# cheneeheng/2s-AGCN

Hardware: AMD Instinct MI355X
Metric: skeleton-clips/sec fwd+bwd, NTU (N,3,300,25,2) (higher is better)
Workload: dtype f32; 1 GPU; AGCN joint-stream NTU-xview shape, full training step (fwd, CE, bwd, grad all-reduce, clip 1.0, SGD nesterov); per_gpu_batch=64, global_batch=64, input=(N,3,300,25,2), parallelism=dp1, bn=per-replica

## Files before the change

### 2s-agcn_amd/csrc/gcn_chain.hip

```cpp
#include "agcn_common.h"
#include "split_f16.h"

namespace {

typedef __bf16 bf16x8 __attribute__((ext_vector_type(8)));
typedef __bf16 bf16x2 __attribute__((ext_vector_type(2)));
typedef float f32x2 __attribute__((ext_vector_type(2)));
typedef unsigned u32x4 __attribute__((ext_vector_type(4)));
typedef f32x4 f32x4_u __attribute__((aligned(4)));

constexpr int CB = 32;

struct ChainArgs {
  const float* in;
  const unsigned short* wp;
  const float* bias;
  float* out;
  const float* adj;
  float* stats;
  const float* add1;
  const float* mask1;
  const float* add2;
  const float* mask2;
  int N, M, K, T, V;
// ... 805 lines not shown
#pragma unroll
        for (int pl = 0; pl < 2; ++pl) af[pl] = *reinterpret_cast<const bf16x8*>(ab + ((pl * 2 + hf) * TM + tm) * 1024);
        acc[tm] = mfma3(af, gb[hf], acc[tm]);
      }
  };

  f32x4 xr[4];
  float dvb[16];
  const int t_first = f0 + wave;
  if (t_first < f1) load_x(t_first, 0, xr);
  __syncthreads();
  const unsigned long long tk_pro = (a.dbg & 8) ? wall_clock64() : 0;
  const unsigned long long ck_pro = (a.dbg & 8) ? clock64() : 0;

  long long ck_st = 0, ck_c = 0, ck_o = 0, ck_e = 0, ck0 = 0;
  int prev_t0 = -1;
  for (int t0 = f0; t0 < f1; t0 += WS_NW) {
    const int t = t0 + wave;
    const bool fvalid = t < f1 && !(a.dbg & 1);
    const bool nvalid_next = (t + WS_NW) < f1 && !(a.dbg & 2);
    f32x16 acc[TM];
#pragma unroll
    for (int tm = 0; tm < TM; ++tm)
#pragma unroll
      for (int j = 0; j < 16; ++j) acc[tm][j] = 0.f;
    if (a.dbg & 8) ck0 = clock64();
    if (fvalid) {
      if (NCB2 > 0) load_p(0, t, dvb);
      bf16x8 xq[2][2];
      u32x4 gw[2][2][2];
      bf16x8 bq[2][2];
      auto load_adj = [&](int i) __attribute__((always_inline)) {
        const unsigned char* aq = adjq + i * 2 * 2048 + (h * 32 + lr) * 16;
#pragma unroll
        for (int ks = 0; ks < 2; ++ks)
#pragma unroll
          for (int pl = 0; pl < 2; ++pl) bq[ks][pl] = *reinterpret_cast<const bf16x8*>(aq + pl * 2048 + ks * 1024);
      };
      auto agg = [&]() __attribute__((always_inline)) {
        f32x16 d;
#pragma unroll
        for (int j = 0; j < 16; ++j) d[j] = 0.f;
#pragma unroll
        for (int ks = 0; ks < 2; ++ks) d = mfma3(xq[ks], bq[ks], d);
        return d;
      };
      auto split_pairs = [&](const float (&dv)[16], int p0, int np, u32x4 (&gwn)[2][2], float sc) __attribute__((always_inline)) {
#pragma unroll
        for (int p = p0; p < p0 + np; ++p) {
          unsigned w0, w1;
          split_pair_f16_mix(dv[2 * p] * sc, dv[2 * p + 1] * sc, w0, w1);
          gwn[p >> 2][0][p & 3] = w0;
          gwn[p >> 2][1][p & 3] = w1;
        }
      };
      auto load_w = [&](int stage, int st, bf16x8 (&af)[2]) __attribute__((always_inline)) {
        const int hf = st / TM, tm = st - hf * TM;
        const unsigned char* ab = wimg + stage * A_IMG + lane * 16;
#pragma unroll
        for (int pl = 0; pl < 2; ++pl) af[pl] = *reinterpret_cast<const bf16x8*>(ab + ((pl * 2 + hf) * TM + tm) * 1024);
      };
      constexpr int NST = 2 * TM;
      constexpr int PP0[4] = {0, 0, 3, 6}, PPN[4] = {0, 3, 3, 2};
      constexpr int QP0[2] = {0, 0}, QPN[2] = {0, 8};
      splitx(xr, xq);
      if (KCB > 1) load_x(t, 1, xr);
      else if (nvalid_next) load_x(t + WS_NW, 0, xr);
      load_adj(0);
      {
        const f32x16 d = agg();
        load_adj(S1 > 1 ? 1 : 0);
        float dv[16];
#pragma unroll
        for (int j = 0; j < 16; ++j) dv[j] = d[j];
        split_pairs(dv, 0, 8, gw[0], 1.f);
      }
      bf16x8 afc[2], afn[2];
      load_w(0, 0, afc);
      __builtin_amdgcn_sched_barrier(0);
#pragma unroll
      for (int s = 0; s < S; ++s) {
        const int sn = s + 1;
        float dv[16];
        if (sn < S1) {
          if (sn % 3 == 0) {
            splitx(xr, xq);
            if (sn / 3 + 1 < KCB) load_x(t, sn / 3 + 1, xr);
            else if (nvalid_next) load_x(t + WS_NW, 0, xr);
          }
          const f32x16 dn = agg();
#pragma unroll
          for (int j = 0; j < 16; ++j) dv[j] = dn[j];
        } else if (sn < S) {
#pragma unroll
          for (int j = 0; j < 16; ++j) dv[j] = dvb[j];
        }
        __builtin_amdgcn_sched_barrier(0);
#pragma unroll
        for (int st = 0; st < NST; ++st) {
          if (!(a.dbg & 32)) {
            if (st + 1 < NST) load_w(s, st + 1, afn);
            else if (sn < S) load_w(sn, 0, afn);
          }
          if (st == NST - 2 && sn + 1 < S1 && !(a.dbg & 64)) load_adj((sn + 1) % 3);
          __builtin_amdgcn_sched_barrier(0);
          {
            const int hf = st / TM, tm = st - hf * TM;
            bf16x8 gbv[2] = {__builtin_bit_cast(bf16x8, gw[s & 1][hf][0]), __builtin_bit_cast(bf16x8, gw[s & 1][hf][1])};
            acc[tm] = mfma3(afc, gbv, acc[tm]);
          }
          if (sn < S && !(a.dbg & 16)) split_pairs(dv, NST == 4 ? PP0[st] : QP0[st], NST == 4 ? PPN[st] : QPN[st], gw[sn & 1], sn < S1 ? 1.f : rs_s);
          afc[0] = afn[0]; afc[1] = afn[1];
          __builtin_amdgcn_sched_barrier(0);
        }
        if (sn >= S1 && sn + 1 < S) load_p(sn + 1 - S1, t, dvb);
        if constexpr (!ROLES) {
          if (prev_t0 >= 0 && s * RB < RPW) {
            if (al16) store_rows_fast(O0, s * RB, prev_t0, WS_NW * V); else store_rows_slow(O0, s * RB, prev_t0, WS_NW * V);
          }
          __builtin_amdgcn_sched_barrier(0);
        }
      }
    }
    if constexpr (!ROLES) {
      if (prev_t0 >= 0 && !fvalid) store_tile(O0, prev_t0, WS_NW * V);
      prev_t0 = t0;
    }
    if (a.dbg & 8) { const long long c = clock64(); ck_st += c - ck0; ck0 = c; }
    if (o_stride == 0) asm volatile("s_waitcnt lgkmcnt(0)\n\ts_barrier" ::: "memory");
    if (a.dbg & 8) { const long long c = clock64(); ck_c += c - ck0; ck0 = c; }
    if (fvalid && lr < V) {
      float* O = O0 + (((t0 - f0) / WS_NW) & 1) * o_stride;
#pragma unroll
      for (int tm = 0; tm < TM; ++tm)
#pragma unroll
        for (int j = 0; j < 16; ++j) O[(tm * 32 + mfma_row(j, h)) * OPf + wave * V + lr] = acc[tm][j];
    }
    if (a.dbg & 8) { asm volatile("s_waitcnt lgkmcnt(0)" ::: "memory"); const long long c = clock64(); ck_o += c - ck0; ck0 = c; }
    asm volatile("s_waitcnt lgkmcnt(0)\n\ts_barrier" ::: "memory");
    if (a.dbg & 8) { const long long c = clock64(); ck_e += c - ck0; ck0 = c; }
  }
  const unsigned long long tk_loop = (a.dbg & 8) ? wall_clock64() : 0;
  if ((a.dbg & 8) && tid == 0) {
    float* o = a.out + blk0 + (long)f0 * V;
    o[0] = (float)(tk_pro - tk_entry); o[1] = (float)(tk_loop - tk_pro); o[2] = (float)(clock64() - ck_pro); o[3] = -12345.f;
    o[4] = (float)ck_st; o[5] = (float)ck_c; o[6] = (float)ck_o; o[7] = (float)ck_e;
  }
  if constexpr (!ROLES) {
    store_tile(O0, prev_t0, min(WS_NW, f1 - prev_t0) * V);
    store_stats();
  }
}

struct ChainGeom {
  int ntiles, ncb, nmb, XP, off_bias;
  size_t smem_bytes, pack_bytes;
};

template <int TM, int NW>
ChainGeom chain_geometry(int V, int T, int M, int K, bool bch = false, int planes = 3) {
  constexpr int BM = TM * 32, FT = NW;
  ChainGeom g;
  g.ntiles = (T + FT - 1) / FT;
  g.ncb = (K + CB - 1) / CB;
  g.nmb = (M + BM - 1) / BM;
  g.XP = (FT * V) | 1;
  const size_t a_img = (size_t)planes * 2 * TM * 1024;
  const size_t xb_bytes = ((size_t)CB * g.XP * 4 + (bch ? 128 : 0) + 15) & ~(size_t)15;
  g.smem_bytes = (bch ? (size_t)3 * planes * 2 * 2 * 32 * 16 : (size_t)3 * 32 * 32 * 4) + xb_bytes + 2 * a_img;
  const size_t epi_bytes = (size_t)BM * ((FT * V) | 1) * 4 + (size_t)NW * 64 * 2 * 4;
  if (epi_bytes > g.smem_bytes) g.smem_bytes = epi_bytes;
  g.smem_bytes = (g.smem_bytes + 15) & ~(size_t)15;
  g.off_bias = (int)g.smem_bytes;
  g.smem_bytes += (size_t)BM * 4;
  g.pack_bytes = (size_t)g.nmb * g.ncb * 3 * a_img;
  return g;
}

struct ChainW2 {
  const float* w;
  long sa_m, sa_c;
};

template <int TM, int VS, int NW, bool F16 = false>
int chain_launch(ChainArgs a, const float* w, long sa_m, long sa_i, long sa_c, const ChainW2& g_w2, void* ws,
                 size_t ws_bytes, hipStream_t stream) {
  constexpr int PL = F16 ? 2 : 3;
  const ChainGeom g = chain_geometry<TM, NW>(a.V, a.T, a.M, a.K, VS == 0, PL);
  if (g.smem_bytes > 160 * 1024) return AGCN_ERR_UNSUPPORTED;
  a.ncb2 = a.in2 ? (a.K2 + CB - 1) / CB : 0;
  const int s_total = 3 * g.ncb + a.ncb2;
  const size_t a_img = (size_t)PL * 2 * TM * 1024;
  const size_t img_bytes = (size_t)g.nmb * s_total * a_img;
  if (img_bytes + (F16 ? 16 : 0) > ws_bytes) return AGCN_ERR_WORKSPACE;
  if constexpr (F16) {
    unsigned* amax = reinterpret_cast<unsigned*>(static_cast<char*>(ws) + img_bytes);
    if (!a.in_absmax) {
      if (int rc = agcn_launch_absmax(a.in, (long)a.N * a.K * a.T * a.V, amax, stream)) return rc;
      a.in_absmax = reinterpret_cast<const float*>(amax);
    }
    if (a.in2 && !a.in2_absmax) {
      if (int rc = agcn_launch_absmax(a.in2, (long)a.N * a.K2 * a.T * a.V, amax + 1, stream)) return rc;
      a.in2_absmax = reinterpret_cast<const float*>(amax + 1);
    }
    if (!a.in2) a.in2_absmax = nullptr;
  }
  a.ntiles = g.ntiles; a.ncb = g.ncb; a.nmb = g.nmb; a.XP = g.XP; a.off_bias = g.off_bias;
  a.wp = (const unsigned short*)ws;
  ChainPackArgs pk;
  pk.w = w; pk.wp = (unsigned short*)ws; pk.M = a.M; pk.K = a.K; pk.ncb = g.ncb;
  pk.sa_m = sa_m; pk.sa_i = sa_i; pk.sa_c = sa_c;
  pk.nsub = 3; pk.s_total = s_total; pk.s_off = 0;
  hipLaunchKernelGGL((chain_pack_kernel<TM, F16>), dim3(g.nmb * g.ncb * 3), dim3(256), 0, stream, pk);
  int rc = agcn_check_launch();
  if (rc) return rc;
  if (a.ncb2 > 0) {
    ChainPackArgs p2;
    p2.w = g_w2.w; p2.wp = (unsigned short*)ws; p2.M = a.M; p2.K = a.K2; p2.ncb = a.ncb2;
    p2.sa_m = g_w2.sa_m; p2.sa_i = 0; p2.sa_c = g_w2.sa_c;
    p2.nsub = 1; p2.s_total = s_total; p2.s_off = 3 * g.ncb;
    hipLaunchKernelGGL((chain_pack_kernel<TM, F16>), dim3(g.nmb * a.ncb2), dim3(256), 0, stream, p2);
    rc = agcn_check_launch();
    if (rc) return rc;
  }
  auto kern = gcn_chain_kernel<TM, VS, NW, F16>;
  static unsigned char lds_ok[AGCN_MAX_DEVICES] = {};
  if (int e = agcn_allow_big_lds_rt(reinterpret_cast<const void*>(kern), lds_ok)) return e;
  hipLaunchKernelGGL(kern, dim3((unsigned)(a.N * g.ntiles * g.nmb)), dim3(NW * 64), g.smem_bytes, stream, a);
  AGCN_NOTE_KERNEL("gcn_chain_kernel<%d, %d, %d, %s>", TM, VS, NW, F16 ? "true" : "false");
  return agcn_check_launch();
}


static inline bool ws_enabled() {
  static const int on = getenv("AGCN_CHAIN_WS") ? atoi(getenv("AGCN_CHAIN_WS")) : 1;
  return on != 0;
}
static inline bool ws_shape_ok(int M, int K, int K2, int V) {
  if (!(agcn_chain_f16x3() && ws_enabled() && V <= 32 && M >= 1 && K > 32)) return false;
  static const int k128 = getenv("AGCN_WS_K128") ? atoi(getenv("AGCN_WS_K128")) : 1;
  return (K <= 64 && K2 >= 0 && K2 <= 96) || (k128 && K <= 128 && K2 == 0 && M > 32);
}

template <int TM, int NCB2, int KCB = 2>
int ws_launch(ChainArgs a, const float* w, long sa_m, long sa_i, long sa_c, const ChainW2& g_w2, void* ws, size_t ws_bytes,
              hipStream_t stream) {
  const WsGeom g = ws_geometry<TM>(a.N, a.M, a.K, a.K2, a.T, a.V);
  if (g.smem_bytes > 160 * 1024) return AGCN_ERR_UNSUPPORTED;
  if (NCB2 > 0 && a.stats) return AGCN_ERR_UNSUPPORTED;
  const size_t img_total = (size_t)g.nmb * g.img_bytes;
  if (img_total + 16 > ws_bytes) return AGCN_ERR_WORKSPACE;
  unsigned* amax = reinterpret_cast<unsigned*>(static_cast<char*>(ws) + img_total);
  if (!a.in_absmax) {
    if (int rc = agcn_launch_absmax(a.in, (long)a.N * a.K * a.T * a.V, amax, stream)) return rc;
    a.in_absmax = reinterpret_cast<const float*>(amax);
  }
  if (a.in2 && !a.in2_absmax) {
    if (int rc = agcn_launch_absmax(a.in2, (long)a.N * a.K2 * a.T * a.V, amax + 1, stream)) return rc;
    a.in2_absmax = reinterpret_cast<const float*>(amax + 1);
  }
  if (!a.in2) a.in2_absmax = nullptr;
  a.ncb = KCB; a.ncb2 = NCB2; a.nmb = g.nmb;
  a.wp = (const unsigned short*)ws;
  const int s_total = 3 * KCB + NCB2;
  ChainPackArgs pk;
  pk.w = w; pk.wp = (unsigned short*)ws; pk.M = a.M; pk.K = a.K; pk.ncb = KCB;
  pk.sa_m = sa_m; pk.sa_i = sa_i; pk.sa_c = sa_c;
  pk.nsub = 3; pk.s_total = s_total; pk.s_off = 0;
  hipLaunchKernelGGL((chain_pack_kernel<TM, true>), dim3(g.nmb * KCB * 3), dim3(256), 0, stream, pk);
  int rc = agcn_check_launch();
  if (rc) return rc;
  if (NCB2 > 0) {
    ChainPackArgs p2;
    p2.w = g_w2.w; p2.wp = (unsigned short*)ws; p2.M = a.M; p2.K = a.K2; p2.ncb = NCB2;
    p2.sa_m = g_w2.sa_m; p2.sa_i = 0; p2.sa_c = g_w2.sa_c;
    p2.nsub = 1; p2.s_total = s_total; p2.s_off = 3 * KCB;
    hipLaunchKernelGGL((chain_pack_kernel<TM, true>), dim3(g.nmb * NCB2), dim3(256), 0, stream, p2);
    rc = agcn_check_launch();
    if (rc) return rc;
  }
  const bool extras = NCB2 > 0 || a.accumulate || a.add1 || a.add2 || a.relu;
  const dim3 grid((unsigned)(a.N * g.nmb * g.nsplit)), block(NCB2 == 0 ? WS_NT : WS_NW * 64);
  if (extras) {
    auto kern = gcn_ws_kernel<TM, KCB, NCB2, true>;
    static unsigned char lds_ok[AGCN_MAX_DEVICES] = {};
    if (int e = agcn_allow_big_lds_rt(reinterpret_cast<const void*>(kern), lds_ok)) return e;
    hipLaunchKernelGGL(kern, grid, block, g.smem_bytes, stream, a, g);
  } else {
    if constexpr (NCB2 == 0) {
      auto kern = gcn_ws_kernel<TM, KCB, 0, false>;
      static unsigned char lds_ok[AGCN_MAX_DEVICES] = {};
      if (int e = agcn_allow_big_lds_rt(reinterpret_cast<const void*>(kern), lds_ok)) return e;
      hipLaunchKernelGGL(kern, grid, block, g.smem_bytes, stream, a, g);
    }
  }
  AGCN_NOTE_KERNEL("gcn_ws_kernel<%d, %d, %d>", TM, KCB, NCB2);
  return agcn_check_launch();
}

template <int TM>
int ws_dispatch(const ChainArgs& a, const float* w, long sa_m, long sa_i, long sa_c, const ChainW2& w2, void* ws,
                size_t ws_bytes, hipStream_t stream) {
  const int ncb2 = a.in2 ? (a.K2 + CB - 1) / CB : 0;
  if (a.K > 64) {
    if constexpr (TM == 2) {
      if (ncb2 == 0) return ws_launch<2, 0, 4>(a, w, sa_m, sa_i, sa_c, w2, ws, ws_bytes, stream);
    }
    return AGCN_ERR_UNSUPPORTED;
  }
  switch (ncb2) {
    case 0: return ws_launch<TM, 0>(a, w, sa_m, sa_i, sa_c, w2, ws, ws_bytes, stream);
    case 1: return ws_launch<TM, 1>(a, w, sa_m, sa_i, sa_c, w2, ws, ws_bytes, stream);
    case 2: return ws_launch<TM, 2>(a, w, sa_m, sa_i, sa_c, w2, ws, ws_bytes, stream);
    case 3: return ws_launch<TM, 3>(a, w, sa_m, sa_i, sa_c, w2, ws, ws_bytes, stream);
  }
  return AGCN_ERR_UNSUPPORTED;
}

template <int TM, int NW>
int chain_dispatch_vs(const ChainArgs& a, const float* w, long sa_m, long sa_i, long sa_c, const ChainW2& w2, void* ws,
                      size_t ws_bytes, hipStream_t stream) {
  static const int f32chain = getenv("AGCN_CHAIN_F32") ? atoi(getenv("AGCN_CHAIN_F32")) : 0;
  if (!f32chain && a.npl == 3 && agcn_chain_f16x3())
    return chain_launch<TM, 0, NW, true>(a, w, sa_m, sa_i, sa_c, w2, ws, ws_bytes, stream);
  if (!f32chain && a.npl == 3) return chain_launch<TM, 0, NW>(a, w, sa_m, sa_i, sa_c, w2, ws, ws_bytes, stream);
  const int vs = (a.V + 1) / 2;
  if (vs == 13) return chain_launch<TM, 13, NW>(a, w, sa_m, sa_i, sa_c, w2, ws, ws_bytes, stream);
  if (vs == 9) return chain_launch<TM, 9, NW>(a, w, sa_m, sa_i, sa_c, w2, ws, ws_bytes, stream);
  return chain_launch<TM, 16, NW>(a, w, sa_m, sa_i, sa_c, w2, ws, ws_bytes, stream);
}


struct DadjArgs {
  const float* dy;
  const unsigned short* wp;
  const float* x;
  float* dpart;
  int N, C, Cout, T, V;
  int ntiles, nkc, nmb, nslots, gpc;
  int npl;
  const float* dy_absmax;
  const float* x_absmax;
  int dbg;
};

struct DadjPackArgs {
  const float* w;
  unsigned short* wp;
  int C3, Cout, nkc;
};

constexpr int KC = 32;

template <int TM, bool F16>
__global__ void __launch_bounds__(256) dadj_pack_kernel(const DadjPackArgs p) {
  constexpr int BM = TM * 32;
  constexpr int PL = F16 ? 2 : 3;
  constexpr int PER_PLANE = 2 * TM * 64 * 8;
  const int kc = blockIdx.x % p.nkc, mb = blockIdx.x / p.nkc;
  unsigned short* dst = p.wp + (long)blockIdx.x * PL * PER_PLANE;
  for (int e = threadIdx.x; e < PER_PLANE / 2; e += 256) {
    const int e2 = e & 3;
    const int lane = (e >> 2) & 63;
    const int r = e >> 8;
    const int tm = r % TM, ks = r / TM;
    const int h = lane >> 5, lr = lane & 31;
    const int m = mb * BM + tm * 32 + lr;
    float v[2];
#pragma unroll
    for (int q = 0; q < 2; ++q) {
      const int o = kc * KC + ks * 16 + h * 8 + 2 * e2 + q;
      v[q] = (m < p.C3 && o < p.Cout) ? p.w[(long)o * p.C3 + m] : 0.f;
    }
    unsigned ph, pm, pl = 0;
    if constexpr (F16) split_pair_f16(v[0] * F16_W_SCALE, v[1] * F16_W_SCALE, ph, pm);
    else split_pair(v[0], v[1], ph, pm, pl);
    const int o2 = ((ks * TM + tm) * 64 + lane) * 8 + 2 * e2;
    *reinterpret_cast<unsigned*>(dst + 0 * PER_PLANE + o2) = ph;
    *reinterpret_cast<unsigned*>(dst + 1 * PER_PLANE + o2) = pm;
    if constexpr (!F16) *reinterpret_cast<unsigned*>(dst + 2 * PER_PLANE + o2) = pl;
  }
}

template <int TM, int NW, bool F16 = false>
__global__ void __launch_bounds__(NW * 64, 2) gcn_dadj_chain_kernel(const DadjArgs a) {
  constexpr int NT = NW * 64, FT = NW, BM = TM * 32;
  constexpr int PL = F16 ? 2 : 3;
  constexpr int A_IMG = PL * 2 * TM * 1024;
  constexpr int A16 = A_IMG / 16;
  constexpr int EA = (A16 + NT - 1) / NT;
  constexpr int BI = (FT * 32 * 4 + NT - 1) / NT;
  extern __shared__ __attribute__((aligned(16))) unsigned char smem[];
  const int V = a.V, T = a.T;
  const int PT = FT * V;
  const int B_IMG = PL * 4 * PT * 16;
  float rs_s = 1.f, rs_inv = 1.f;
  const bool red16 = F16 && a.x_absmax != nullptr;
  float xs = 1.f, xinv = 1.f;
  if constexpr (F16) {
    if (red16) {
      f16_range_scale_of<F16_ADJ_TARGET>(*a.dy_absmax, rs_s, rs_inv);
      f16_range_scale_of<14>(*a.x_absmax, xs, xinv);
    } else {
      f16_range_scale(a.dy_absmax, rs_s, rs_inv);
    }
    rs_inv *= F16_W_INV * xinv;
  }
  unsigned char* abuf = smem;
  unsigned char* bbuf = smem + 2 * A_IMG;

  const int tid = threadIdx.x, lane = tid & 63;
  const int wave = __builtin_amdgcn_readfirstlane(tid >> 6);
  const int lr = lane & 31, h = lane >> 5;
  const int bid = xcd_remap(blockIdx.x, gridDim.x);
  const int mbk = bid % a.nmb;
  const int nt_id = bid / a.nmb;
  const int n = nt_id / a.ntiles, tile_id = nt_id - n * a.ntiles;
  const int m0 = mbk * BM;
  const int isub = mbk / a.gpc, c0 = (mbk - isub * a.gpc) * BM;
  const int t0 = tile_id * FT;
  const int t = t0 + wave;
  const bool fvalid = t < T;
  const int plen = min(FT, T - t0) * V;
  const long P = (long)T * V;
  const int S = a.nkc;

  f32x16 acc[TM];
#pragma unroll
  for (int tm = 0; tm < TM; ++tm)
#pragma unroll
    for (int j = 0; j < 16; ++j) acc[tm][j] = 0.f;

  u32x4 ra[EA];
  f32x4 rb[8];
  const u32x4* wp4 = reinterpret_cast<const u32x4*>(a.wp) + (long)mbk * S * A16;
  const int npiece = (PT + 3) >> 2, ntask = 4 * npiece;
  const float* dy_end = a.dy + (long)a.N * a.Cout * P;
  auto issue = [&](int s) __attribute__((always_inline)) {
    const u32x4* src = wp4 + (long)s * A16;
#pragma unroll
    for (int u = 0; u < EA; ++u) ra[u] = src[min(tid + u * NT, A16 - 1)];
    int tk = tid;
    asm volatile("" : "+v"(tk));
    if (tk < ntask) {
      const int og = tk / npiece, pos = (tk - og * npiece) * 4;
      const int o0 = s * KC + og * 8;
      const float* src2 = a.dy + ((long)n * a.Cout + min(o0, a.Cout - 8)) * P + (long)t0 * V + pos;
      if (src2 + 7 * P + 4 <= dy_end) {
#pragma unroll
        for (int e = 0; e < 8; ++e) rb[e] = *reinterpret_cast<const f32x4_u*>(src2 + (long)e * P);
      } else {
#pragma unroll
        for (int e = 0; e < 8; ++e)
#pragma unroll
          for (int q = 0; q < 4; ++q) {
            const float* pq = src2 + (long)e * P + q;
            rb[e][q] = (pq < dy_end) ? *pq : 0.f;
          }
      }
    }
  };
  auto commit = [&](int s) __attribute__((always_inline)) {
    u32x4* dst = reinterpret_cast<u32x4*>(abuf + (s & 1) * A_IMG);
#pragma unroll
    for (int u = 0; u < EA; ++u)
      if (tid + u * NT < A16) dst[tid + u * NT] = ra[u];
    unsigned char* bd = bbuf + (s & 1) * B_IMG;
    int tk = tid;
    asm volatile("" : "+v"(tk));
    if (tk < ntask) {
      const int og = tk / npiece, pos = (tk - og * npiece) * 4;
#pragma unroll
      for (int q = 0; q < 4; ++q) {
        u32x4 ph, pm, pl;
#pragma unroll
        for (int e2 = 0; e2 < 4; ++e2) {
          unsigned q0, q1, q2 = 0;
          if constexpr (F16) split_pair_f16(rb[2 * e2][q] * rs_s, rb[2 * e2 + 1][q] * rs_s, q0, q1);
          else split_pair(rb[2 * e2][q], rb[2 * e2 + 1][q], q0, q1, q2);
          ph[e2] = q0; pm[e2] = q1; pl[e2] = q2;
        }
        if (pos + q < PT) {
// ... 29 lines not shown
#pragma unroll
      for (int ks = 0; ks < 2; ++ks) {
        bf16x8 b[PL];
#pragma unroll
        for (int pl = 0; pl < PL; ++pl)
          b[pl] = *reinterpret_cast<const bf16x8*>(bb + (((pl * 2 + ks) * 2 + h) * PT + bpos) * 16);
#pragma unroll
        for (int tm = 0; tm < TM; ++tm) {
          const bf16x8 a0 = *reinterpret_cast<const bf16x8*>(ab + ((0 * 2 + ks) * TM + tm) * 1024);
          const bf16x8 a1 = *reinterpret_cast<const bf16x8*>(ab + ((1 * 2 + ks) * TM + tm) * 1024);
          if constexpr (F16) {
            acc[tm] = __builtin_amdgcn_mfma_f32_32x32x16_f16(__builtin_bit_cast(f16x8, a1), __builtin_bit_cast(f16x8, b[0]), acc[tm], 0, 0, 0);
            acc[tm] = __builtin_amdgcn_mfma_f32_32x32x16_f16(__builtin_bit_cast(f16x8, a0), __builtin_bit_cast(f16x8, b[1]), acc[tm], 0, 0, 0);
            acc[tm] = __builtin_amdgcn_mfma_f32_32x32x16_f16(__builtin_bit_cast(f16x8, a0), __builtin_bit_cast(f16x8, b[0]), acc[tm], 0, 0, 0);
            continue;
          }
          const bf16x8 a2 = *reinterpret_cast<const bf16x8*>(ab + ((PL - 1) * 2 + ks) * TM * 1024 + tm * 1024);
          if (a.npl == 3) {
            acc[tm] = __builtin_amdgcn_mfma_f32_32x32x16_bf16(a2, b[0], acc[tm], 0, 0, 0);
            acc[tm] = __builtin_amdgcn_mfma_f32_32x32x16_bf16(a0, b[PL - 1], acc[tm], 0, 0, 0);
            acc[tm] = __builtin_amdgcn_mfma_f32_32x32x16_bf16(a1, b[1], acc[tm], 0, 0, 0);
            acc[tm] = __builtin_amdgcn_mfma_f32_32x32x16_bf16(a1, b[0], acc[tm], 0, 0, 0);
            acc[tm] = __builtin_amdgcn_mfma_f32_32x32x16_bf16(a0, b[1], acc[tm], 0, 0, 0);
          }
          acc[tm] = __builtin_amdgcn_mfma_f32_32x32x16_bf16(a0, b[0], acc[tm], 0, 0, 0);
        }
      }
    }
    __syncthreads();
  }

  f32x16 d;
#pragma unroll
  for (int j = 0; j < 16; ++j) d[j] = 0.f;
  if (fvalid && !(a.dbg & 1)) {
    float xb[2][16];
#pragma unroll
    for (int tm = 0; tm < TM; ++tm) {
      if (tm + 1 < TM) load_x(tm + 1, xb[(tm + 1) & 1]);
      if (F16 && red16) {
#pragma unroll
        for (int ks = 0; ks < 2; ++ks) {
          u32x4 ah, al, bh, bl;
#pragma unroll
          for (int e2 = 0; e2 < 4; ++e2) {
            const int j = 8 * ks + 2 * e2;
            float x0 = (tm == 0) ? xa0[j] : xb[tm & 1][j];
            float x1 = (tm == 0) ? xa0[j + 1] : xb[tm & 1][j + 1];
            x0 = (lr < V) ? x0 * xs : 0.f;
            x1 = (lr < V) ? x1 * xs : 0.f;
            unsigned p0, p1, q0, q1;
            split_pair_f16_mix(x0, x1, p0, p1);
            split_pair_f16_mix(acc[tm][j], acc[tm][j + 1], q0, q1);
            ah[e2] = p0; al[e2] = p1; bh[e2] = q0; bl[e2] = q1;
          }
          d = __builtin_amdgcn_mfma_f32_32x32x16_f16(__builtin_bit_cast(f16x8, al), __builtin_bit_cast(f16x8, bh), d, 0, 0, 0);
          d = __builtin_amdgcn_mfma_f32_32x32x16_f16(__builtin_bit_cast(f16x8, ah), __builtin_bit_cast(f16x8, bl), d, 0, 0, 0);
          d = __builtin_amdgcn_mfma_f32_32x32x16_f16(__builtin_bit_cast(f16x8, ah), __builtin_bit_cast(f16x8, bh), d, 0, 0, 0);
        }
        continue;
      }
#pragma unroll
      for (int j = 0; j < 16; ++j) {
        const float xv = (tm == 0) ? xa0[j] : xb[tm & 1][j];
        d = mfma32((lr < V) ? xv : 0.f, acc[tm][j], d);
      }
    }
  }
  const int VV = V * V;
  float* red = reinterpret_cast<float*>(smem);
#pragma unroll
  for (int j = 0; j < 16; ++j) {
    const int u = mfma_row(j, h);
    if (u < V && lr < V) red[wave * VV + u * V + lr] = F16 ? d[j] * rs_inv : d[j];
  }
  __syncthreads();
  const int slot = tile_id * a.gpc + (mbk - isub * a.gpc);
  float* dst = a.dpart + (((long)n * 3 + isub) * a.nslots + slot) * VV;
  for (int e = tid; e < VV; e += NT) {
    float sum = 0.f;
#pragma unroll
    for (int w2 = 0; w2 < NW; ++w2) sum += red[w2 * VV + e];
    dst[e] = sum;
  }
}

template <int TM, int NW, bool F16 = false>
int dadj_chain_launch(DadjArgs a, const float* wcat, void* ws, size_t ws_bytes, hipStream_t stream) {
  constexpr int BM = TM * 32, FT = NW;
  constexpr int PL = F16 ? 2 : 3;
  a.ntiles = (a.T + FT - 1) / FT;
  a.nkc = (a.Cout + KC - 1) / KC;
  a.gpc = a.C / BM;
  a.nmb = 3 * a.gpc;
  a.nslots = a.ntiles * a.gpc;
  const size_t a_img = (size_t)PL * 2 * TM * 1024;
  const size_t b_img = (size_t)PL * 4 * FT * a.V * 16;
  size_t smem_bytes = 2 * a_img + 2 * b_img;
  const size_t epi = (size_t)NW * a.V * a.V * 4;
  if (epi > smem_bytes) smem_bytes = epi;
  if (smem_bytes > 160 * 1024) return AGCN_ERR_UNSUPPORTED;
  const size_t pack_bytes = (size_t)a.nmb * a.nkc * a_img;
  if (pack_bytes + (F16 ? 16 : 0) > ws_bytes) return AGCN_ERR_WORKSPACE;
  a.wp = (const unsigned short*)ws;
  if constexpr (F16) {
    if (!a.dy_absmax) {
      unsigned* amax = reinterpret_cast<unsigned*>(static_cast<char*>(ws) + pack_bytes);
      if (int rc = agcn_launch_absmax(a.dy, (long)a.N * a.Cout * a.T * a.V, amax, stream)) return rc;
      a.dy_absmax = reinterpret_cast<const float*>(amax);
    }
    static const int red16 = getenv("AGCN_DADJ_RED16") ? atoi(getenv("AGCN_DADJ_RED16")) : 1;
    if (!red16) {
      a.x_absmax = nullptr;
    } else if (!a.x_absmax) {
      unsigned* amax = reinterpret_cast<unsigned*>(static_cast<char*>(ws) + pack_bytes) + 1;
      if (int rc = agcn_launch_absmax(a.x, (long)a.N * a.C * a.T * a.V, amax, stream)) return rc;
      a.x_absmax = reinterpret_cast<const float*>(amax);
    }
  }
  DadjPackArgs pk;
  pk.w = wcat; pk.wp = (unsigned short*)ws; pk.C3 = 3 * a.C; pk.Cout = a.Cout; pk.nkc = a.nkc;
  hipLaunchKernelGGL((dadj_pack_kernel<TM, F16>), dim3(a.nmb * a.nkc), dim3(256), 0, stream, pk);
  int rc = agcn_check_launch();
  if (rc) return rc;
  auto kern = gcn_dadj_chain_kernel<TM, NW, F16>;
  static unsigned char lds_ok[AGCN_MAX_DEVICES] = {};
  if (int e = agcn_allow_big_lds_rt(reinterpret_cast<const void*>(kern), lds_ok)) return e;
  hipLaunchKernelGGL(kern, dim3((unsigned)(a.N * a.ntiles * a.nmb)), dim3(NW * 64), smem_bytes, stream, a);
  return agcn_check_launch();
}

}

static inline int chain_tm(int M) { return (M % 128 == 0) ? 4 : (M <= 32 ? 1 : 2); }

static inline int chain_waves() {
  static int nw = 0;
  if (!nw) {
    const char* e = getenv("AGCN_CHAIN_WAVES");
    nw = (e && atoi(e) == 8) ? 8 : 4;
  }
  return nw;
}

int agcn_chain_f16x3() {
  static const int on = getenv("AGCN_CHAIN_F16X3") ? atoi(getenv("AGCN_CHAIN_F16X3")) : 1;
  return on && agcn_npl() == 3;
}

bool agcn_gcn_chain_supported(int M, int K, int V) { return M >= 1 && K >= 1 && V <= 32; }

int agcn_gcn_chain_tiles(int T) { return (T + chain_waves() - 1) / chain_waves(); }

int agcn_gcn_chain_stats_slots(int N, int M, int K, int T, int V) {
  if (ws_shape_ok(M, K, 0, V)) {
    const WsGeom g = (M <= 32) ? ws_geometry<1>(N, M, K, 0, T, V) : ws_geometry<2>(N, M, K, 0, T, V);
    if (g.smem_bytes <= 160 * 1024) return N * g.nsplit;
  }
  return N * agcn_gcn_chain_tiles(T);
}

size_t agcn_gcn_chain_workspace(int M, int K, int K2, int T, int V) {
  (void)T; (void)V;
  const int tm = chain_tm(M), bm = 32 * tm;
  const size_t a_img = (size_t)3 * 2 * tm * 1024;
  return (size_t)((M + bm - 1) / bm) * (3 * ((K + CB - 1) / CB) + (K2 + CB - 1) / CB) * a_img;
}

int agcn_gcn_chain(int mode, const float* in, const float* adj, const float* wcat, const float* bias, float* out,
                   float* stats_part, int accumulate, const float* add1, const float* mask1, const float* add2,
                   const float* mask2, int mask_bits, const float* in2, const float* w2, int K2, void* ws, size_t ws_bytes,
                   int N, int C, int Cout, int T, int V, hipStream_t stream, int relu, int w2_rows_are_outputs,
                   const float* in_absmax, const float* in2_absmax) {
  ChainArgs a = {};
  a.relu = relu;
  a.in_absmax = in_absmax; a.in2_absmax = in2_absmax;
  a.npl = agcn_npl();
  { static const int dbg = getenv("AGCN_GC_DBG") ? atoi(getenv("AGCN_GC_DBG")) : 0; a.dbg = dbg; }
  a.in2 = (in2 && w2 && K2 > 0) ? in2 : nullptr;
  a.K2 = a.in2 ? K2 : 0;
  ChainW2 cw2 = {w2, 1, 0};
  a.in = in; a.adj = adj; a.bias = bias; a.out = out; a.stats = stats_part;
  a.accumulate = accumulate; a.add1 = add1; a.mask1 = mask1; a.add2 = add2; a.mask2 = mask2; a.mask_bits = mask_bits;
  a.N = N; a.T = T; a.V = V;
  long sa_m, sa_i, sa_c;
  if (mode == 0) { a.M = Cout; a.K = C; a.adj_t = 0; sa_m = 3L * C; sa_i = C; sa_c = 1; }
  else           { a.M = C; a.K = Cout; a.adj_t = 1; sa_m = 1; sa_i = C; sa_c = 3L * C; }
  cw2.sa_c = a.M;
  if (w2_rows_are_outputs) { cw2.sa_m = a.K2; cw2.sa_c = 1; }
  if (!a.dbg && ws_shape_ok(a.M, a.K, a.K2, V)) {
    if (const char* e = getenv("AGCN_WS_DBG")) a.dbg = atoi(e);
    const int rc = (a.M <= 32) ? ws_dispatch<1>(a, wcat, sa_m, sa_i, sa_c, cw2, ws, ws_bytes, stream)
                               : ws_dispatch<2>(a, wcat, sa_m, sa_i, sa_c, cw2, ws, ws_bytes, stream);
    if (rc != AGCN_ERR_UNSUPPORTED) return rc;
  }
  if (chain_waves() == 8 && chain_tm(a.M) != 1) {
    if (chain_tm(a.M) == 4) return chain_dispatch_vs<4, 8>(a, wcat, sa_m, sa_i, sa_c, cw2, ws, ws_bytes, stream);
    return chain_dispatch_vs<2, 8>(a, wcat, sa_m, sa_i, sa_c, cw2, ws, ws_bytes, stream);
  }
  if (chain_tm(a.M) == 4) return chain_dispatch_vs<4, 4>(a, wcat, sa_m, sa_i, sa_c, cw2, ws, ws_bytes, stream);
  if (chain_tm(a.M) == 1) return chain_dispatch_vs<1, 4>(a, wcat, sa_m, sa_i, sa_c, cw2, ws, ws_bytes, stream);
  return chain_dispatch_vs<2, 4>(a, wcat, sa_m, sa_i, sa_c, cw2, ws, ws_bytes, stream);
}

constexpr int DADJ_NW = 8;
constexpr int DADJ_NW64 = 4;
bool agcn_gcn_dadj_chain_supported(int C, int V) { return C >= 64 && C % 64 == 0 && V <= 32; }

int agcn_gcn_dadj_chain_slots(int C, int T) {
  const int bm = (C % 128 == 0) ? 128 : 64;
  const int nw = (bm == 128) ? DADJ_NW : DADJ_NW64;
  return ((T + nw - 1) / nw) * (C / bm);
}

size_t agcn_gcn_dadj_chain_workspace(int C, int Cout) {
  const int bm = (C % 128 == 0) ? 128 : 64;
  return (size_t)(3 * C / bm) * ((Cout + KC - 1) / KC) * 3 * 2 * (bm / 32) * 1024;
}

int agcn_gcn_dadj_chain(const float* dy, const float* wcat, const float* x, float* dadj_part, void* ws, size_t ws_bytes,
                        int N, int C, int Cout, int T, int V, hipStream_t stream, const float* dy_absmax,
                        const float* x_absmax) {
  DadjArgs a = {};
  a.npl = agcn_npl();
  a.dy = dy; a.x = x; a.dpart = dadj_part; a.N = N; a.C = C; a.Cout = Cout; a.T = T; a.V = V;
  a.dy_absmax = dy_absmax;
  a.x_absmax = x_absmax;
  if (const char* e = getenv("AGCN_DADJ_DBG")) a.dbg = atoi(e);
  static const int f16 = getenv("AGCN_DADJ_F16X3") ? atoi(getenv("AGCN_DADJ_F16X3")) : 1;
  if (agcn_chain_f16x3() && f16) {
    if (C % 128 == 0) return dadj_chain_launch<4, DADJ_NW, true>(a, wcat, ws, ws_bytes, stream);
    return dadj_chain_launch<2, DADJ_NW64, true>(a, wcat, ws, ws_bytes, stream);
  }
  if (C % 128 == 0) return dadj_chain_launch<4, DADJ_NW>(a, wcat, ws, ws_bytes, stream);
  return dadj_chain_launch<2, DADJ_NW64>(a, wcat, ws, ws_bytes, stream);
}
```

Before: 1043 clips/s.

## Add full-height GCN chain kernel covering all output channels per block

Adds a new gcn_chain_fh kernel in which each block computes every output channel (up to 256) for a small time tile. Weights are streamed through a three-stage LDS ring with global_load_lds DMA, and the input times adjacency product is done once per channel block instead of once per M-block. It is selected by default for M between 65 and 256 when the work-split path does not apply. The kernel also brings a new epilogue with finer stats slots (one per 4 frames) and a workspace sizing change. The aim is to stop recomputing the graph aggregation across M-blocks and to get better weight reuse, at the cost of more LDS per block and more register pressure.

After: 1055 clips/s (median of 6 runs). +1.1%, better.

```diff
diff --git a/2s-agcn_amd/csrc/gcn_chain.hip b/2s-agcn_amd/csrc/gcn_chain.hip
--- a/2s-agcn_amd/csrc/gcn_chain.hip
+++ b/2s-agcn_amd/csrc/gcn_chain.hip
@@ -981,6 +981,316 @@
   }
 }
 
+constexpr int FH_R = 3;
+constexpr int FH_ADJ = 3 * 2 * 2 * 2 * 32 * 16;
+constexpr int FH_SF = 4;
+
+template <int TM> constexpr int fh_img() { return 2 * 2 * TM * 1024; }
+template <int TM, int NW> constexpr int fh_npass() { return (TM == 8 && NW == 8) ? 2 : 1; }
+template <int NW> constexpr int fh_rg() { return NW == 8 ? 2 : 4; }
+
+template <int TM, int NW>
+__global__ void __launch_bounds__(NW * 64, NW == 8 ? 2 : 1) gcn_chain_fh_kernel(const ChainArgs a) {
+  constexpr int NT = NW * 64, FT = NW, BM = TM * 32;
+  constexpr int FH_IMG = fh_img<TM>();
+  constexpr int PPW = (FH_IMG / 1024) / NW;
+  constexpr int NPASS = fh_npass<TM, NW>(), TMP = TM / NPASS, BMP = BM / NPASS;
+  constexpr int SG = FT / FH_SF;
+  constexpr int XB = FT / 2;
+  extern __shared__ __attribute__((aligned(16))) unsigned char smem[];
+  unsigned char* ring = smem;
+  unsigned char* adjq = smem + FH_R * FH_IMG;
+
+  const int tid = threadIdx.x, lane = tid & 63;
+  const int wave = __builtin_amdgcn_readfirstlane(tid >> 6);
+  const int lr = lane & 31, h = lane >> 5;
+  const int bid = xcd_remap(blockIdx.x, gridDim.x);
+  const int n = bid / a.ntiles, tile_id = bid - n * a.ntiles;
+  const int V = a.V, T = a.T;
+  const int t0 = tile_id * FT, t = t0 + wave;
+  const bool fvalid = t < T;
+  const int xlen = min(FT, T - t0) * V;
+  const long P = (long)T * V;
+  const int S1 = 3 * a.ncb, S = S1 + a.ncb2;
+  float rs_s = 1.f, rs_inv = 1.f;
+  {
+    float mx = a.in_absmax ? *a.in_absmax : 0.f;
+    if (a.in2_absmax) mx = fmaxf(mx, *a.in2_absmax);
+    f16_range_scale_of<F16_ADJ_TARGET>(mx, rs_s, rs_inv);
+    rs_inv *= F16_W_INV;
+  }
+
+  const unsigned char* wsrc = reinterpret_cast<const unsigned char*>(a.wp) + lane * 16;
+  const unsigned ring_lds = (unsigned)(unsigned long)(__attribute__((address_space(3))) unsigned char*)ring;
+  auto dma_stage = [&](int s) __attribute__((always_inline)) {
+    const unsigned char* src = wsrc + (long)s * FH_IMG;
+    const unsigned dst = ring_lds + (unsigned)((s % FH_R) * FH_IMG);
+#pragma unroll
+    for (int u = 0; u < PPW; ++u) {
+      const int piece = wave + u * NW;
+      asm volatile("global_load_lds_dwordx4 %0, off" :: "v"(src + piece * 1024),
+                   "{m0}"(__builtin_amdgcn_readfirstlane(dst + piece * 1024)) : "memory");
+    }
+  };
+  dma_stage(0);
+  if (S > 1) dma_stage(1);
+
+  float* bias_s = reinterpret_cast<float*>(smem + a.off_bias);
+  for (int e = tid; e < BM; e += NT) bias_s[e] = (a.bias && e < a.M) ? a.bias[e] : 0.f;
+  {
+    const float* adjn = a.adj + (long)n * 3 * V * V;
+    for (int e = tid; e < 3 * 2 * 2 * 32 * 4; e += NT) {
+      const int e2 = e & 3, col = (e >> 2) & 31, hh = (e >> 7) & 1, ks = (e >> 8) & 1, i = e >> 9;
+      float v[2];
+#pragma unroll
+      for (int q = 0; q < 2; ++q) {
+        const int u = 16 * ks + 8 * hh + 2 * e2 + q;
+        const bool ok = u < V && col < V;
+        const int gi = ok ? (a.adj_t ? ((i * V + col) * V + u) : ((i * V + u) * V + col)) : 0;
+        const float tv = adjn[gi];
+        v[q] = ok ? tv : 0.f;
+      }
+      unsigned p0, p1;
+      split_pair_f16(v[0], v[1], p0, p1);
+      const int o = (((ks * 2 + hh) * 32) + col) * 16 + e2 * 4;
+      *reinterpret_cast<unsigned*>(adjq + (i * 2 + 0) * 2048 + o) = p0;
+      *reinterpret_cast<unsigned*>(adjq + (i * 2 + 1) * 2048 + o) = p1;
+    }
+  }
+
+  const __amdgpu_buffer_rsrc_t rx = __builtin_amdgcn_make_buffer_rsrc(
+      const_cast<float*>(a.in + (long)n * a.K * P), 0, (int)((long)a.K * P * 4), 0x00020000);
+  const __amdgpu_buffer_rsrc_t rx2 = __builtin_amdgcn_make_buffer_rsrc(
+      const_cast<float*>(a.in2 ? a.in2 + (long)n * a.K2 * P : a.in), 0, a.in2 ? (int)((long)a.K2 * P * 4) : 0, 0x00020000);
+  auto load_x = [&](int cb, f32x4 (&xc)[4]) __attribute__((always_inline)) {
+    const int off = (int)(((long)min(cb * CB + lr, a.K - 1) * P + (long)t * V + 8 * h) * 4);
+#pragma unroll
+    for (int q = 0; q < 4; ++q)
+      xc[q] = __builtin_bit_cast(f32x4, __builtin_amdgcn_raw_buffer_load_b128(rx, off + ((q >> 1) * 16 + (q & 1) * 4) * 4, 0, 0));
+  };
+  auto load_p = [&](int s2, float (&dv)[16]) __attribute__((always_inline)) {
+    const int pos = (t * V + min(lr, V - 1)) * 4;
+#pragma unroll
+    for (int j = 0; j < 16; ++j) {
+      const int c2 = min(s2 * CB + (j & 3) + 8 * (j >> 2) + 4 * h, a.K2 - 1);
+      dv[j] = __builtin_bit_cast(float, __builtin_amdgcn_raw_buffer_load_b32(rx2, (int)((long)c2 * P * 4) + pos, 0, 0));
+    }
+  };
+  auto mfma3 = [&](const bf16x8 (&x)[2], const bf16x8 (&y)[2], f32x16 c) __attribute__((always_inline)) {
+    c = __builtin_amdgcn_mfma_f32_32x32x16_f16(__builtin_bit_cast(f16x8, x[1]), __builtin_bit_cast(f16x8, y[0]), c, 0, 0, 0);
+    c = __builtin_amdgcn_mfma_f32_32x32x16_f16(__builtin_bit_cast(f16x8, x[0]), __builtin_bit_cast(f16x8, y[1]), c, 0, 0, 0);
+    c = __builtin_amdgcn_mfma_f32_32x32x16_f16(__builtin_bit_cast(f16x8, x[0]), __builtin_bit_cast(f16x8, y[0]), c, 0, 0, 0);
+    return c;
+  };
+  auto split8 = [&](const float (&v)[8], bf16x8 (&q)[2], float sc) __attribute__((always_inline)) {
+    u32x4 w0, w1;
+#pragma unroll
+    for (int e2 = 0; e2 < 4; ++e2) {
+      unsigned p0, p1;
+      split_pair_f16_mix(v[2 * e2] * sc, v[2 * e2 + 1] * sc, p0, p1);
+      w0[e2] = p0; w1[e2] = p1;
+    }
+    q[0] = __builtin_bit_cast(bf16x8, w0);
+    q[1] = __builtin_bit_cast(bf16x8, w1);
+  };
+
+  f32x16 acc[TM];
+#pragma unroll
+  for (int tm = 0; tm < TM; ++tm)
+#pragma unroll
+    for (int j = 0; j < 16; ++j) acc[tm][j] = 0.f;
+  f32x4 xr[4];
+  float dvb[16];
+  if (fvalid) {
+    if (a.ncb > 0) load_x(0, xr);
+    else load_p(0, dvb);
+  }
+  asm volatile("s_waitcnt vmcnt(0)" ::: "memory");
+  __syncthreads();
+
+  bf16x8 xq[2][2];
+  long long tk0 = 0, tk_stage = 0, tk_mat = 0, tk_bar = 0;
+  const long long tk_begin = (a.dbg & 8) ? clock64() : 0;
+  for (int s = 0; s < S; ++s) {
+    const bool plain = s >= S1;
+    const int cb = plain ? 0 : s / 3, i = plain ? 0 : s - cb * 3;
+    if (a.dbg & 8) tk0 = clock64();
+    bf16x8 gb[2][2];
+    if (fvalid && !(a.dbg & 1)) {
+      float dv[16];
+      if (!plain) {
+        if (i == 0) {
+#pragma unroll
+          for (int ks = 0; ks < 2; ++ks) {
+            float xv[8];
+#pragma unroll
+            for (int e = 0; e < 4; ++e) { xv[e] = xr[2 * ks][e]; xv[4 + e] = xr[2 * ks + 1][e]; }
+            split8(xv, xq[ks], rs_s);
+          }
+          if (cb + 1 < a.ncb) load_x(cb + 1, xr);
+        }
+        if (s + 1 == S1 && a.ncb2 > 0) load_p(0, dvb);
+        f32x16 d;
+#pragma unroll
+        for (int j = 0; j < 16; ++j) d[j] = 0.f;
+        const unsigned char* aq = adjq + i * 2 * 2048 + (h * 32 + lr) * 16;
+#pragma unroll
+        for (int ks = 0; ks < 2; ++ks) {
+          bf16x8 bq[2];
+#pragma unroll
+          for (int pl = 0; pl < 2; ++pl) bq[pl] = *reinterpret_cast<const bf16x8*>(aq + pl * 2048 + ks * 1024);
+          d = mfma3(xq[ks], bq, d);
+        }
+#pragma unroll
+        for (int j = 0; j < 16; ++j) dv[j] = d[j];
+      } else {
+#pragma unroll
+        for (int j = 0; j < 16; ++j) dv[j] = dvb[j] * rs_s;
+        if (s + 1 < S) load_p(s + 1 - S1, dvb);
+      }
+#pragma unroll
+      for (int hf = 0; hf < 2; ++hf) {
+        float gv[8];
+#pragma unroll
+        for (int e = 0; e < 8; ++e) gv[e] = dv[8 * hf + e];
+        split8(gv, gb[hf], 1.f);
+      }
+    }
+    if (s + 2 < S && !(a.dbg & 2)) dma_stage(s + 2);
+    if (a.dbg & 8) { const long long c = clock64(); tk_stage += c - tk0; tk0 = c; }
+    if (fvalid && !(a.dbg & 1)) {
+      const unsigned char* ab = ring + (s % FH_R) * FH_IMG + lane * 16;
+      auto load_w = [&](bf16x8 (&af)[2], int step) __attribute__((always_inline)) {
+        const int hf = step / TM, tm = step - hf * TM;
+#pragma unroll
+        for (int pl = 0; pl < 2; ++pl) af[pl] = *reinterpret_cast<const bf16x8*>(ab + ((pl * 2 + hf) * TM + tm) * 1024);
+      };
+      bf16x8 afc[2];
+      load_w(afc, 0);
+      __builtin_amdgcn_sched_group_barrier(0x100, 2, 0);
+#pragma unroll
+      for (int step = 0; step < 2 * TM; ++step) {
+        const int hf = step / TM, tm = step - hf * TM;
+        bf16x8 afn[2];
+        if (step + 1 < 2 * TM) load_w(afn, step + 1);
+        acc[tm] = mfma3(afc, gb[hf], acc[tm]);
+        if (step + 1 < 2 * TM) {
+          __builtin_amdgcn_sched_group_barrier(0x100, 2, 0);
+          afc[0] = afn[0]; afc[1] = afn[1];
+        }
+        __builtin_amdgcn_sched_group_barrier(0x008, 3, 0);
+      }
+    }
+    if (a.dbg & 8) { const long long c = clock64(); tk_mat += c - tk0; tk0 = c; }
+    if (s + 2 < S && !(a.dbg & 2)) asm volatile("s_waitcnt vmcnt(%0)\n\ts_waitcnt lgkmcnt(0)\n\ts_barrier" :: "n"(PPW) : "memory");
+    else asm volatile("s_waitcnt vmcnt(0)\n\ts_waitcnt lgkmcnt(0)\n\ts_barrier" ::: "memory");
+    if (a.dbg & 8) { const long long c = clock64(); tk_bar += c - tk0; }
+  }
+  const long long tk_loop_end = (a.dbg & 8) ? clock64() : 0;
+
+  constexpr int RG = fh_rg<NW>(), NG = BMP / (NW * RG);
+  const bool has_extra = a.accumulate || a.add1 || a.add2;
+  float* tile = reinterpret_cast<float*>(smem);
+  const int TP = (FT * V) | 1;
+  auto epi_pass = [&](auto pass_c) __attribute__((always_inline)) {
+    constexpr int pass = decltype(pass_c)::value;
+    const int mp = pass * BMP;
+    if (pass > 0) __syncthreads();
+    float ex[2][5][RG][XB];
+    auto row_base = [&](int k, int g) __attribute__((always_inline)) {
+      const int m = min(mp + (k * NW + wave) * RG + g, a.M - 1);
+      return (((long)n * a.M + m) * T + t0) * V;
+    };
+    auto load_extras = [&](int k, float (&e)[5][RG][XB]) __attribute__((always_inline)) {
+#pragma unroll
+      for (int g = 0; g < RG; ++g) {
+        const long base = row_base(k, g);
+#pragma unroll
+        for (int u = 0; u < XB; ++u) {
+          const int q = lane + 64 * u;
+          const long idx = base + ((q < xlen) ? q : 0);
+          if (a.accumulate) e[0][g][u] = a.out[idx];
+          if (a.add1) e[1][g][u] = a.add1[idx];
+          if (a.mask1) e[2][g][u] = mask_load(a.mask1, idx, a.mask_bits);
+          if (a.add2) e[3][g][u] = a.add2[idx];
+          if (a.mask2) e[4][g][u] = mask_load(a.mask2, idx, a.mask_bits);
+        }
+      }
+    };
+    if (has_extra) load_extras(0, ex[0]);
+    if (fvalid && lr < V) {
+#pragma unroll
+      for (int tm = 0; tm < TMP; ++tm)
+#pragma unroll
+        for (int j = 0; j < 16; ++j)
+          tile[(tm * 32 + mfma_row(j, h)) * TP + wave * V + lr] = acc[pass * TMP + tm][j] * rs_inv;
+    }
+    __syncthreads();
+    if (a.stats) {
+      float* red = tile + BMP * TP;
+      const int r = tid % BMP;
+      const float bval = bias_s[mp + r];
+      for (int part = tid / BMP; part < SG * 2; part += NT / BMP) {
+        const int sg = part >> 1, sl = part & 1;
+        const int q0 = sg * FH_SF * V, q1 = min(xlen, q0 + FH_SF * V);
+        float bsum = 0.f, bsq = 0.f;
+#pragma unroll 8
+        for (int q = q0 + sl; q < q1; q += 2) {
+          const float y = tile[r * TP + q] + bval;
+          bsum += y;
+          bsq += y * y;
+        }
+        red[(part * 2 + 0) * BMP + r] = bsum;
+        red[(part * 2 + 1) * BMP + r] = bsq;
+      }
+      __syncthreads();
+      const int nslot = (T + FH_SF - 1) / FH_SF;
+      for (int e = tid; e < SG * 2 * BMP; e += NT) {
+        const int sg = e / (2 * BMP), k = (e / BMP) & 1, ml = e % BMP;
+        const int st = tile_id * SG + sg;
+        if (st >= nslot || mp + ml >= a.M) continue;
+        float sum = 0.f;
+#pragma unroll
+        for (int sl = 0; sl < 2; ++sl) sum += red[((sg * 2 + sl) * 2 + k) * BMP + ml];
+        a.stats[(((long)n * nslot + st) * 2 + k) * a.M + mp + ml] = sum;
+      }
+    }
+#pragma unroll
+    for (int k = 0; k < NG; ++k) {
+      const int r0 = (k * NW + wave) * RG;
+      if (mp + r0 >= a.M) break;
+      if (has_extra && k + 1 < NG) load_extras(k + 1, ex[(k + 1) & 1]);
+#pragma unroll
+      for (int g = 0; g < RG; ++g) {
+        const int m = mp + r0 + g;
+        if (m >= a.M) break;
+        const long base = row_base(k, g);
+        const float bval = bias_s[m];
+#pragma unroll
+        for (int u = 0; u < XB; ++u) {
+          const int q = lane + 64 * u;
+          float v = tile[(r0 + g) * TP + min(q, TP - 1)] + bval;
+          if (a.accumulate) v += ex[k & 1][0][g][u];
+          const long midx = base + ((q < xlen) ? q : 0);
+          if (a.add1) v += (!a.mask1 || mask_pass(ex[k & 1][2][g][u], midx, a.mask_bits)) ? ex[k & 1][1][g][u] : 0.f;
+          if (a.add2) v += (!a.mask2 || mask_pass(ex[k & 1][4][g][u], midx, a.mask_bits)) ? ex[k & 1][3][g][u] : 0.f;
+          if (a.relu) v = fmaxf(v, 0.f);
+          if (q < xlen) a.out[base + q] = v;
+        }
+      }
+    }
+  };
+  epi_pass(std::integral_constant<int, 0>{});
+  if constexpr (NPASS > 1) epi_pass(std::integral_constant<int, 1>{});
+  if ((a.dbg & 8) && blockIdx.x == gridDim.x / 2 && tid == 0) {
+    const long long tk_end = clock64();
+    float* o = a.out + (long)n * a.M * P + (long)t0 * V;
+    o[0] = (float)(tk_loop_end - tk_begin); o[1] = (float)tk_stage; o[2] = (float)tk_mat; o[3] = (float)tk_bar;
+    o[4] = (float)(tk_end - tk_loop_end); o[5] = (float)S;
+    o[6] = -12345.f;
+  }
+}
+
 struct ChainGeom {
   int ntiles, ncb, nmb, XP, off_bias;
   size_t smem_bytes, pack_bytes;
@@ -1146,10 +1456,15 @@
   return AGCN_ERR_UNSUPPORTED;
 }
 
+static inline int chain_f32() {
+  static const int on = getenv("AGCN_CHAIN_F32") ? atoi(getenv("AGCN_CHAIN_F32")) : 0;
+  return on;
+}
+
 template <int TM, int NW>
 int chain_dispatch_vs(const ChainArgs& a, const float* w, long sa_m, long sa_i, long sa_c, const ChainW2& w2, void* ws,
                       size_t ws_bytes, hipStream_t stream) {
-  static const int f32chain = getenv("AGCN_CHAIN_F32") ? atoi(getenv("AGCN_CHAIN_F32")) : 0;
+  const int f32chain = chain_f32();
   if (!f32chain && a.npl == 3 && agcn_chain_f16x3())
     return chain_launch<TM, 0, NW, true>(a, w, sa_m, sa_i, sa_c, w2, ws, ws_bytes, stream);
   if (!f32chain && a.npl == 3) return chain_launch<TM, 0, NW>(a, w, sa_m, sa_i, sa_c, w2, ws, ws_bytes, stream);
@@ -1157,6 +1472,69 @@
   if (vs == 13) return chain_launch<TM, 13, NW>(a, w, sa_m, sa_i, sa_c, w2, ws, ws_bytes, stream);
   if (vs == 9) return chain_launch<TM, 9, NW>(a, w, sa_m, sa_i, sa_c, w2, ws, ws_bytes, stream);
   return chain_launch<TM, 16, NW>(a, w, sa_m, sa_i, sa_c, w2, ws, ws_bytes, stream);
+}
+
+struct FhGeom {
+  int ntiles, ncb, off_bias;
+  size_t smem_bytes;
+};
+
+template <int TM, int NW>
+static inline FhGeom fh_geometry(int K, int T, int V) {
+  constexpr int BMP = TM * 32 / fh_npass<TM, NW>();
+  FhGeom g;
+  g.ntiles = (T + NW - 1) / NW;
+  g.ncb = (K + CB - 1) / CB;
+  const size_t loop_bytes = (size_t)FH_R * fh_img<TM>() + FH_ADJ;
+  const size_t epi_bytes = (size_t)BMP * ((NW * V) | 1) * 4 + (size_t)(NW / FH_SF) * 2 * 2 * BMP * 4;
+  g.off_bias = (int)(((loop_bytes > epi_bytes ? loop_bytes : epi_bytes) + 15) & ~(size_t)15);
+  g.smem_bytes = (size_t)g.off_bias + TM * 32 * 4;
+  return g;
+}
+
+template <int TM, int NW>
+int fh_launch(ChainArgs a, const float* w, long sa_m, long sa_i, long sa_c, const ChainW2& g_w2, void* ws, size_t ws_bytes,
+              hipStream_t stream) {
+  const FhGeom g = fh_geometry<TM, NW>(a.K, a.T, a.V);
+  if (g.smem_bytes > 160 * 1024 || a.M > TM * 32) return AGCN_ERR_UNSUPPORTED;
+  a.ncb2 = a.in2 ? (a.K2 + CB - 1) / CB : 0;
+  const int s_total = 3 * g.ncb + a.ncb2;
+  const size_t img_bytes = (size_t)s_total * fh_img<TM>();
+  if (img_bytes + 16 > ws_bytes) return AGCN_ERR_WORKSPACE;
+  unsigned* amax = reinterpret_cast<unsigned*>(static_cast<char*>(ws) + img_bytes);
+  if (!a.in_absmax) {
+    if (int rc = agcn_launch_absmax(a.in, (long)a.N * a.K * a.T * a.V, amax, stream)) return rc;
+    a.in_absmax = reinterpret_cast<const float*>(amax);
+  }
+  if (a.in2 && !a.in2_absmax) {
+    if (int rc = agcn_launch_absmax(a.in2, (long)a.N * a.K2 * a.T * a.V, amax + 1, stream)) return rc;
+    a.in2_absmax = reinterpret_cast<const float*>(amax + 1);
+  }
+  if (!a.in2) a.in2_absmax = nullptr;
+  a.ntiles = g.ntiles; a.ncb = g.ncb; a.nmb = 1; a.off_bias = g.off_bias;
+  a.wp = (const unsigned short*)ws;
+  ChainPackArgs pk;
+  pk.w = w; pk.wp = (unsigned short*)ws; pk.M = a.M; pk.K = a.K; pk.ncb = g.ncb;
+  pk.sa_m = sa_m; pk.sa_i = sa_i; pk.sa_c = sa_c;
+  pk.nsub = 3; pk.s_total = s_total; pk.s_off = 0;
+  hipLaunchKernelGGL((chain_pack_kernel<TM, true>), dim3(g.ncb * 3), dim3(256), 0, stream, pk);
+  int rc = agcn_check_launch();
+  if (rc) return rc;
+  if (a.ncb2 > 0) {
+    ChainPackArgs p2;
+    p2.w = g_w2.w; p2.wp = (unsigned short*)ws; p2.M = a.M; p2.K = a.K2; p2.ncb = a.ncb2;
+    p2.sa_m = g_w2.sa_m; p2.sa_i = 0; p2.sa_c = g_w2.sa_c;
+    p2.nsub = 1; p2.s_total = s_total; p2.s_off = 3 * g.ncb;
+    hipLaunchKernelGGL((chain_pack_kernel<TM, true>), dim3(a.ncb2), dim3(256), 0, stream, p2);
+    rc = agcn_check_launch();
+    if (rc) return rc;
+  }
+  auto kern = gcn_chain_fh_kernel<TM, NW>;
+  static unsigned char lds_ok[AGCN_MAX_DEVICES] = {};
+  if (int e = agcn_allow_big_lds_rt(reinterpret_cast<const void*>(kern), lds_ok)) return e;
+  hipLaunchKernelGGL(kern, dim3((unsigned)(a.N * g.ntiles)), dim3(NW * 64), g.smem_bytes, stream, a);
+  AGCN_NOTE_KERNEL("gcn_chain_fh_kernel<%d, %d>", TM, NW);
+  return agcn_check_launch();
 }
 
 
@@ -1492,19 +1870,46 @@
 
 int agcn_gcn_chain_tiles(int T) { return (T + chain_waves() - 1) / chain_waves(); }
 
+static inline int fh_mode() {
+  static const int on = getenv("AGCN_CHAIN_FH") ? atoi(getenv("AGCN_CHAIN_FH")) : 2;
+  return on;
+}
+static inline int fh_waves() {
+  static const int nw = (getenv("AGCN_CHAIN_FH_WAVES") && atoi(getenv("AGCN_CHAIN_FH_WAVES")) == 4) ? 4 : 8;
+  return nw;
+}
+static inline int gc_dbg() {
+  static const int dbg = getenv("AGCN_GC_DBG") ? atoi(getenv("AGCN_GC_DBG")) : 0;
+  return dbg;
+}
+
+enum { CHAIN_WS, CHAIN_FH, CHAIN_TILE };
+struct ChainPlan { int kind, slots; };
+static ChainPlan chain_plan(int N, int M, int K, int K2, int T, int V, int dbg, bool stats) {
+  if (!dbg && ws_shape_ok(M, K, K2, V) && !(K2 > 0 && stats)) {
+    const WsGeom g = (M <= 32) ? ws_geometry<1>(N, M, K, K2, T, V) : ws_geometry<2>(N, M, K, K2, T, V);
+    if (g.smem_bytes <= 160 * 1024) return {CHAIN_WS, N * g.nsplit};
+  }
+  if (agcn_chain_f16x3() && !chain_f32() && M <= 256 && M > (fh_mode() >= 2 ? 64 : 128) && fh_mode() >= 1 && V <= 32) {
+    const bool w4 = fh_waves() == 4;
+    const FhGeom g = (M > 128) ? (w4 ? fh_geometry<8, 4>(K, T, V) : fh_geometry<8, 8>(K, T, V))
+                               : (w4 ? fh_geometry<4, 4>(K, T, V) : fh_geometry<4, 8>(K, T, V));
+    if (g.smem_bytes <= 160 * 1024) return {CHAIN_FH, N * ((T + FH_SF - 1) / FH_SF)};
+  }
+  return {CHAIN_TILE, N * agcn_gcn_chain_tiles(T)};
+}
+
 int agcn_gcn_chain_stats_slots(int N, int M, int K, int T, int V) {
-  if (ws_shape_ok(M, K, 0, V)) {
-    const WsGeom g = (M <= 32) ? ws_geometry<1>(N, M, K, 0, T, V) : ws_geometry<2>(N, M, K, 0, T, V);
-    if (g.smem_bytes <= 160 * 1024) return N * g.nsplit;
-  }
-  return N * agcn_gcn_chain_tiles(T);
+  return chain_plan(N, M, K, 0, T, V, gc_dbg(), true).slots;
 }
 
 size_t agcn_gcn_chain_workspace(int M, int K, int K2, int T, int V) {
   (void)T; (void)V;
   const int tm = chain_tm(M), bm = 32 * tm;
-  const size_t a_img = (size_t)3 * 2 * tm * 1024;
-  return (size_t)((M + bm - 1) / bm) * (3 * ((K + CB - 1) / CB) + (K2 + CB - 1) / CB) * a_img;
+  const size_t stages = (size_t)(3 * ((K + CB - 1) / CB) + (K2 + CB - 1) / CB);
+  const size_t tile = (size_t)((M + bm - 1) / bm) * stages * 3 * 2 * tm * 1024;
+  const size_t fh = stages * fh_img<8>() + 16;
+  return tile > fh ? tile : fh;
 }
 
 int agcn_gcn_chain(int mode, const float* in, const float* adj, const float* wcat, const float* bias, float* out,
@@ -1516,7 +1921,7 @@
   a.relu = relu;
   a.in_absmax = in_absmax; a.in2_absmax = in2_absmax;
   a.npl = agcn_npl();
-  { static const int dbg = getenv("AGCN_GC_DBG") ? atoi(getenv("AGCN_GC_DBG")) : 0; a.dbg = dbg; }
+  a.dbg = gc_dbg();
   a.in2 = (in2 && w2 && K2 > 0) ? in2 : nullptr;
   a.K2 = a.in2 ? K2 : 0;
   ChainW2 cw2 = {w2, 1, 0};
@@ -1528,11 +1933,18 @@
   else           { a.M = C; a.K = Cout; a.adj_t = 1; sa_m = 1; sa_i = C; sa_c = 3L * C; }
   cw2.sa_c = a.M;
   if (w2_rows_are_outputs) { cw2.sa_m = a.K2; cw2.sa_c = 1; }
-  if (!a.dbg && ws_shape_ok(a.M, a.K, a.K2, V)) {
+  const ChainPlan plan = chain_plan(N, a.M, a.K, a.K2, T, V, a.dbg, stats_part != nullptr);
+  if (plan.kind == CHAIN_WS) {
     if (const char* e = getenv("AGCN_WS_DBG")) a.dbg = atoi(e);
-    const int rc = (a.M <= 32) ? ws_dispatch<1>(a, wcat, sa_m, sa_i, sa_c, cw2, ws, ws_bytes, stream)
-                               : ws_dispatch<2>(a, wcat, sa_m, sa_i, sa_c, cw2, ws, ws_bytes, stream);
-    if (rc != AGCN_ERR_UNSUPPORTED) return rc;
+    return (a.M <= 32) ? ws_dispatch<1>(a, wcat, sa_m, sa_i, sa_c, cw2, ws, ws_bytes, stream)
+                       : ws_dispatch<2>(a, wcat, sa_m, sa_i, sa_c, cw2, ws, ws_bytes, stream);
+  }
+  if (plan.kind == CHAIN_FH) {
+    if (a.M > 128)
+      return (fh_waves() == 4) ? fh_launch<8, 4>(a, wcat, sa_m, sa_i, sa_c, cw2, ws, ws_bytes, stream)
+                               : fh_launch<8, 8>(a, wcat, sa_m, sa_i, sa_c, cw2, ws, ws_bytes, stream);
+    return (fh_waves() == 4) ? fh_launch<4, 4>(a, wcat, sa_m, sa_i, sa_c, cw2, ws, ws_bytes, stream)
+                             : fh_launch<4, 8>(a, wcat, sa_m, sa_i, sa_c, cw2, ws, ws_bytes, stream);
   }
   if (chain_waves() == 8 && chain_tm(a.M) != 1) {
     if (chain_tm(a.M) == 4) return chain_dispatch_vs<4, 8>(a, wcat, sa_m, sa_i, sa_c, cw2, ws, ws_bytes, stream);
```
